# mfkiwl/conan-slam

Hardware: AMD Instinct MI355X
Metric: ekf_update_steps_per_sec (higher is better)
Workload: dtype f32

## Files before the change

conan_slam_amd/_capi.py:

```python
from __future__ import annotations

import ctypes as C
import os
import re

_HERE = os.path.dirname(os.path.abspath(__file__))
LIB_PATH = os.path.join(_HERE, "lib", "libcslam_hip.so")
HEADER_PATH = os.path.join(_HERE, "..", "include", "cslam.h")

OK, ERR_BAD_ARG, ERR_CAPACITY, ERR_HIP, ERR_NO_DEVICE, ERR_ALLOC = 0, 1, 2, 3, 4, 5
FACTOR_OK, FACTOR_FALLBACK, FACTOR_ZEROED, FACTOR_SKIPPED, FACTOR_BAD_IDF, FACTOR_INTERNAL = 0, 1, 2, 4, 8, 16
FACTOR_HEADING_SKIPPED = 32
F32, F64 = 0, 1
Q_LOWER_CHOL_GAIN, Q_PREDICT_NM4, Q_REF_EXACT, Q_TEXTBOOK = 1, 2, 3, 0
STAGE_GATHER, STAGE_FACTOR, STAGE_GAIN, STAGE_DOWNDATE, N_STAGES = 0, 1, 2, 3, 4
STAGE_NAMES = ["gather", "factor", "gain", "downdate"]


class CslamError(RuntimeError):
    def __init__(self, code: int, msg: str):
        super().__init__(f"cslam status {code}: {msg}")
        self.code = code


BATCH_MC_SYMBOLS = ("cslam_ekf_batch_predict_each", "cslam_ekf_batch_get_poses")

LANDMARK_SYMBOLS = ("cslam_ekf_get_landmarks", "cslam_ekf_batch_get_landmarks")
_PROTOTYPES = {
    "cslam_ekf_get_landmarks": [C.c_void_p, C.c_int, C.c_int, C.c_void_p, C.c_void_p, C.c_void_p],
    "cslam_ekf_batch_get_landmarks": [C.c_void_p, C.c_int, C.c_int, C.c_void_p, C.c_void_p, C.c_void_p],
    "cslam_ekf_rows_launches": [C.c_void_p, C.POINTER(C.c_longlong)],
    "cslam_sim_batch_create": [C.c_void_p, C.c_int, C.c_int, C.POINTER(C.c_longlong), C.c_int, C.POINTER(C.c_void_p)],
    "cslam_sim_batch_destroy": [C.c_void_p],
    "cslam_sim_batch_scan": [C.c_void_p, C.c_void_p, C.c_double, C.c_void_p, C.c_longlong, C.POINTER(C.c_int),
                             C.POINTER(C.c_int), C.POINTER(C.c_int)],
    "cslam_sim_batch_get_scan": [C.c_void_p, C.c_int, C.c_void_p, C.c_void_p, C.c_void_p, C.c_void_p],
    "cslam_sim_batch_get_table": [C.c_void_p, C.c_void_p],
    "cslam_sim_batch_set_table": [C.c_void_p, C.c_void_p],
    "cslam_ekf_batch_update_scan": [C.c_void_p, C.c_void_p, C.c_void_p],
    "cslam_ekf_batch_augment_scan": [C.c_void_p, C.c_void_p, C.c_void_p],
    "cslam_pf_best_particle": [C.c_void_p, C.c_int, C.POINTER(C.c_int)] + [C.c_void_p] * 5,
    "cslam_pf_estimate": [C.c_void_p, C.POINTER(C.c_double), C.POINTER(C.c_double)] + [C.c_void_p] * 4,
    "cslam_pf_get_all_features": [C.c_void_p, C.c_void_p],
    "cslam_pf_best_particle_sharded": [C.c_void_p, C.c_void_p, C.c_int, C.POINTER(C.c_longlong)] + [C.c_void_p] * 5,
    "cslam_pf_estimate_sharded": [C.c_void_p, C.c_void_p, C.POINTER(C.c_double), C.POINTER(C.c_double)]
                                 + [C.c_void_p] * 4,
}
PF_ESTIMATE_SYMBOLS = tuple(k for k in _PROTOTYPES if k.startswith("cslam_pf_"))
PF_PICK_MAX, PF_PICK_MIN = 0, 1
SIM_BATCH_SYMBOLS = tuple(k for k in _PROTOTYPES if "sim_batch" in k or k.endswith("_scan"))

SCORE_FIELD_NAMES = ("POSE_N", "POSE_BAD", "POSE_IN", "POSE_ERR2", "POSE_EPHI2", "POSE_NEES",
                     "LM_N", "LM_BAD", "LM_IN", "LM_ERR2", "LM_NEES")
(SCORE_POSE_N, SCORE_POSE_BAD, SCORE_POSE_IN, SCORE_POSE_ERR2, SCORE_POSE_EPHI2, SCORE_POSE_NEES,
 SCORE_LM_N, SCORE_LM_BAD, SCORE_LM_IN, SCORE_LM_ERR2, SCORE_LM_NEES) = range(len(SCORE_FIELD_NAMES))
SCORE_FIELDS = len(SCORE_FIELD_NAMES)
_PROTOTYPES.update({
    "cslam_ekf_batch_score_reset": [C.c_void_p, C.c_int, C.c_double, C.c_double],
    "cslam_ekf_batch_score_set_truth": [C.c_void_p, C.c_void_p, C.c_int],
    "cslam_ekf_batch_score": [C.c_void_p, C.c_void_p],
    "cslam_ekf_batch_score_scan": [C.c_void_p, C.c_void_p, C.c_void_p],
    "cslam_ekf_batch_get_scores": [C.c_void_p, C.c_void_p, C.c_void_p, C.c_int, C.POINTER(C.c_int),
                                   C.POINTER(C.c_longlong)],
})
SCORE_SYMBOLS = tuple(k for k in _PROTOTYPES if "_score" in k)


_PROTOTYPES.update({
    "cslam_pf_associate": [C.c_void_p, C.c_void_p, C.c_int, C.c_void_p, C.c_double, C.c_double],
    "cslam_pf_get_association": [C.c_void_p, C.c_void_p, C.c_void_p, C.c_void_p],
    "cslam_pf_sample_proposal_assoc": [C.c_void_p, C.c_void_p, C.c_int, C.c_void_p, C.c_void_p, C.c_void_p, C.c_double],
    "cslam_pf_feature_update_assoc": [C.c_void_p, C.c_void_p, C.c_int, C.c_void_p, C.c_void_p],
    "cslam_pf_get_stream": [C.c_void_p, C.POINTER(C.c_void_p)],
})
PF_ASSOC_SYMBOLS = tuple(k for k in _PROTOTYPES if k.startswith("cslam_pf_") and "assoc" in k)
PF_ASSOC_FEAT_CHUNK, PF_ASSOC_OBS_CHUNK = 32, 8


def declared_symbols(header_path: str = HEADER_PATH):
    text = open(header_path).read()
    text = re.sub(r"/\*.*?\*/", "", text, flags=re.S)
    return sorted(set(re.findall(r"\b(cslam_[a-z0-9_]+)\s*\(", text)))


# ... 49 lines not shown
```

conan_slam_amd/csrc/cslam_ekf.hip:

```cpp
#include <hip/hip_runtime.h>

#include <algorithm>
#include <atomic>
#include <cfloat>
#include <cmath>
#include <cstdint>
#include <cstdlib>
#include <new>
#include <string>
#include <thread>
#include <vector>

#include "cslam_common.hpp"
#include "device_owners.hpp"
#include "ekf_kernels.hpp"
#include "ekf_kernels_fast.hpp"
#include "ekf_landmark_kernels.hpp"
#include "ekf_lookahead.hpp"
#include "ekf_options.hpp"
#include "ekf_pending_store.hpp"
#include "ekf_pgemm_limbs.hpp"
#include "ekf_pose_kernels.hpp"
#include "ekf_staging.hpp"
#include "host_linalg.hpp"
// ... 16 lines not shown
    for (int i = threadIdx.x; i < 3 * j.m; i += 128)
    {
        if (i < 2 * j.m)
        {
            j.Z_out[i] = j.Z[i];
        }
        else
        {
            j.idf_out[i - 2 * j.m] = j.idf[i - 2 * j.m];
        }
    }
    return true;
}
__global__ void __launch_bounds__(128) ekf_la_wide_f32(LaWideArgs a)
{
    if (la_wide_snapshot(a.snap))
    {
        return;
    }
    ekf_la_wide_body<1, 0>(a);
}
__global__ void __launch_bounds__(128) ekf_la_wide_f32_k64(LaWideArgs a)
{
    if (la_wide_snapshot(a.snap))
    {
        return;
    }
    ekf_la_wide_body<1, 64>(a);
}

__global__ void __launch_bounds__(128) ekf_la_wide_f32_k64m(LaWideArgs a, float* WT)
{
    if (la_wide_snapshot(a.snap))
    {
        return;
    }
    ekf_la_wide_body<1, 64, 1>(a, WT);
}

__global__ void __launch_bounds__(256) ekf_la_blocks_mirror_kernel(LaPrepArgs<float> a, LaMirrorArgs mi)
{
    ekf_la_blocks_mirror_body(a, mi);
}
}

using namespace cslam;

namespace
{

std::atomic<int>& g_engines = ::cslam::live_engines();

constexpr size_t kLdsBudget    = 150 * 1024;

struct EkfBase
{
    explicit EkfBase(const EkfOptions& o) : opt(o) {}
    virtual ~EkfBase() {}
    const EkfOptions opt;
    int         dtype    = CSLAM_F32;
    int         device   = 0;
    int         quirks   = CSLAM_Q_REF_EXACT;
    int         nmax     = 0;
    int         ncap     = 0;
    int         ldp      = 0;
    int         n        = 3;
    int         sync_mode = 1;
    int         pgemm_wgs     = 0;
    Stream      stream_own, stream_b_own, stream_f_own;
    hipStream_t stream   = nullptr;
    hipStream_t stream_b = nullptr;
    long long   la_windows = 0;
    long long   stage_launches = 0;
    long long   rows_launches = 0;

    virtual int init()                                                                        = 0;
    virtual int set_state(const void* X, int n, const void* P, int ldp)                        = 0;
    virtual int get_state(void* X, void* P, int ldp)                                           = 0;
    virtual int get_x(void* X, int cap)                                                        = 0;
    virtual int get_landmarks(int first, int count, void* x, void* pll, void* pvl)             = 0;
    virtual int trace(double* tr)                                                              = 0;
    virtual int predict(double v, double swa, const void* Q, double wb, double dt)             = 0;
    virtual int update(const void* Z, int m, const void* R, const int* idf, int batch, bool on_device) = 0;
    virtual int augment(const void* Z, int q, const void* R)                                   = 0;
    virtual int observe_heading(double phi, int use)                                           = 0;
    virtual int associate(const void* Z, int m, const void* R, double g1, double g2, int* idf_out, int* kind) = 0;
    virtual int factor_status(int* flags, int clear)                                           = 0;
    virtual int set_profiling(int on)                                                          = 0;
    virtual int get_stage_times(double* ms, int* launches)                                     = 0;
    virtual int debug_last_update(void* PHT, void* S, void* G, void* W1, void* V, int* k)      = 0;
    virtual int set_deferred(int max_cols)                                                     = 0;
    virtual int do_flush()                                                                     = 0;
    virtual int resolve_predict()                                                              = 0;
    virtual int sync_all()                                                                     = 0;
    virtual int la_drain()                                                                     = 0;
};

template <typename T>
struct Ekf : EkfBase
{
    using EkfBase::EkfBase;
    DevBuf<T>   dX, dP;
    DevBuf<T>   dPv;
    DevBuf<int> dPoseDone;
    DevBuf<int> dSign;
    DevBuf<T>   dLm;
    PendingCols pend;
    Event      ev_a2b, ev_pgemm;
    T*         last_slot = nullptr;
    struct Workspace
    {
        DevBuf<T> dPHT, dS, dG, dGt, dV, dt_, dScrS, dScrG;
        DevBuf<T> dSub;
        DevBuf<T> dM;
        DevBuf<T> dU;
        DevBuf<T> dWv;
        DevBuf<T> dY;

        int alloc(int ldp, int newk, int wcap, hipStream_t st)
        {
            const size_t kk = (size_t)newk * (newk + 1);
            int          rc = dPHT.alloc_zeroed((size_t)ldp * newk, st);
            if (rc || (rc = dS.alloc(kk)) || (rc = dG.alloc(kk)) || (rc = dSub.alloc((size_t)(3 + 64) * 64)) ||
                (rc = dM.alloc((size_t)3 * 128)) || (rc = dGt.alloc(kk)) || (rc = dScrS.alloc(kk)) ||
                (rc = dScrG.alloc(kk)) || (rc = dV.alloc((size_t)newk)) || (rc = dt_.alloc((size_t)newk)) ||
                (rc = dU.alloc((size_t)newk)) || (rc = dWv.alloc_zeroed((size_t)3 * newk, st)) || (wcap > 0 &&
                (rc = dY.alloc((size_t)newk * wcap))))
// ... 1882 lines not shown
                }
            }
        }
        if (V)
        {
            CSLAM_HIP_TRY(hipMemcpyAsync(V, dbgV ? dbgV : ws.dV.get(), (size_t)k * sizeof(T), hipMemcpyDeviceToHost,
                                         stream));
        }
        CSLAM_HIP_TRY(hipStreamSynchronize(stream));
        return CSLAM_OK;
    }
};

template <typename T>
int Ekf<T>::ensure_tile_list(int tiles)
{
    if (tiles == tiles_built)
    {
        return CSLAM_OK;
    }
    std::vector<int2> h;
    h.reserve((size_t)tiles * (tiles + 1) / 2);
    for (int tj = 0; tj < tiles; tj++)
    {
        for (int ti = tj; ti < tiles; ti++)
        {
            h.push_back(make_int2(ti, tj));
        }
    }
    if (int rc = sync_all())
    {
        return rc;
    }
    DevBuf<int2> list;
    CSLAM_TRY(list.alloc(h.size()));
    dTiles = std::move(list);
    CSLAM_HIP_TRY(hipMemcpy(dTiles.get(), h.data(), h.size() * sizeof(int2), hipMemcpyHostToDevice));
    tiles_built = tiles;
    n_sym_tiles = (int)h.size();
    return CSLAM_OK;
}

template <>
int Ekf<float>::launch_downdate(const float* W, int k, hipStream_t stream)
{
    const int tiles = round_up(n, kTile) / kTile;
    const int k8    = round_up(k, 8);
    int rc = ensure_tile_list(tiles);
    if (rc)
    {
        return rc;
    }
    const dim3 block(256);
    int G = std::min(n_sym_tiles, std::max(1, 2 * (num_cus - la_cus) - (opt.pipeline ? opt.pgemm_spare : 0)));
    if (pgemm_wgs > 0)
    {
        G = std::min(G, pgemm_wgs);
    }
    const bool nt = opt.psym_nt >= 0 ? opt.psym_nt != 0 : (size_t)n_sym_tiles * 65536 > ((size_t)230 << 20);
    if (limbs_take(k8))
    {
        const int    nch  = k8 <= 64 ? 4 : (k8 <= 96 ? 6 : (k8 <= 128 ? 8 : (k8 <= 192 ? 12 : 16)));
        const int    kgs  = 2 * nch;
        const int    rows = round_up(n, kTile);
        const size_t need = (size_t)2 * 3 * kgs * rows * 16;
        if (need > wb_bytes)
        {
            CSLAM_HIP_TRY(hipStreamSynchronize(stream));
            const size_t  cap = (size_t)2 * 3 * 32 * round_up(ncap, kTile) * 16;
            DevBuf<uint4> wb;
            CSLAM_TRY(wb.alloc(cap / sizeof(uint4)));
            dWb      = std::move(wb);
            wb_bytes = cap;
        }
        if ((rc = ensure_tiles_morton(tiles, stream)))
        {
            return rc;
        }
        hipLaunchKernelGGL(ekf_limb_split_kernel, dim3((rows + 255) / 256, kgs), dim3(256), 0, stream, W, ldp, k, rows, kgs,
                           dWb.get());
        limb_parity ^= 1;
#define CSLAM_LAUNCH_PSYM5(MODE, NCH, NP, RR)                                                                          \
    do                                                                                                                 \
    {                                                                                                                  \
        static bool attr_set = false;                                                                                  \
        if (!attr_set)                                                                                                 \
        {                                                                                                              \
            CSLAM_HIP_TRY(hipFuncSetAttribute(reinterpret_cast<const void*>(&ekf_downdate_psym5_bf16<MODE, NCH, NP, RR>), \
                                              hipFuncAttributeMaxDynamicSharedMemorySize, 150 * 1024));               \
            attr_set = true;                                                                                           \
        }                                                                                                              \
        hipLaunchKernelGGL((ekf_downdate_psym5_bf16<MODE, NCH, NP, RR>), dim3(G), block, (size_t)RR * 24576, stream, dP.get(), ldp, \
                           (const uint4*)dWb.get(), rows, (const int2*)dTilesM.get(), (const int*)dSegOff.get(), dTicketX.get() + 8 * limb_parity,  \
                           dTicketX.get() + 8 * (limb_parity ^ 1));                                                          \
    } while (0)
#define CSLAM_LAUNCH_PSYM5R(NCH, RR)                                                                                   \
    do                                                                                                                 \
    {                                                                                                                  \
        if (opt.pgemm_limbs == 6)                                                                                          \
        {                                                                                                              \
            if (nt) { CSLAM_LAUNCH_PSYM5(1, NCH, 6, RR); } else { CSLAM_LAUNCH_PSYM5(0, NCH, 6, RR); }                 \
        }                                                                                                              \
        else                                                                                                           \
        {                                                                                                              \
            if (nt) { CSLAM_LAUNCH_PSYM5(1, NCH, 9, RR); } else { CSLAM_LAUNCH_PSYM5(0, NCH, 9, RR); }                 \
        }                                                                                                              \
    } while (0)
        switch (nch)
        {
        case 4: CSLAM_LAUNCH_PSYM5R(4, 3); break;
        case 6: CSLAM_LAUNCH_PSYM5R(6, 3); break;
        case 8: CSLAM_LAUNCH_PSYM5R(8, 3); break;
        case 12: CSLAM_LAUNCH_PSYM5R(12, 3); break;
        default: CSLAM_LAUNCH_PSYM5R(16, 3); break;
        }
#undef CSLAM_LAUNCH_PSYM5R
#undef CSLAM_LAUNCH_PSYM5
    }
    else if (k8 <= 128 && opt.lower && ldp < 32768)
    {
        launch_parity++;
        const bool xq = opt.xcd_queues != 0 && G >= 64;
        if (xq)
        {
            if ((rc = ensure_tiles_morton(tiles, stream)))
            {
                return rc;
            }
            limb_parity ^= 1;
        }
#define CSLAM_LAUNCH_PSYM4(MODE, NCH, KC)                                                                             \
    hipLaunchKernelGGL((ekf_downdate_psym4_f32<MODE, NCH, KC>), dim3(G), block, 0, stream, dP.get(), ldp, W, ldp, k,         \
                       xq ? (const int2*)dTilesM.get() : (const int2*)dTiles.get(), n_sym_tiles,                                  \
                       xq ? dTicketX.get() + 8 * limb_parity : dTicket.get() + (launch_parity & 1),                              \
                       xq ? dTicketX.get() + 8 * (limb_parity ^ 1) : dTicket.get() + ((launch_parity + 1) & 1),                  \
                       (unsigned long long*)nullptr, xq ? (const int*)dSegOff.get() : (const int*)nullptr, 0u, 0u, 0u, 0u,           \
                       la_sig_add ? la.done.get() : (unsigned*)nullptr, la_sig_add, 1, 0)
        if (k8 <= 64)
        {
            if (nt) { CSLAM_LAUNCH_PSYM4(1, 2, 32); } else { CSLAM_LAUNCH_PSYM4(0, 2, 32); }
        }
        else if (k8 <= 96)
        {
            if (nt) { CSLAM_LAUNCH_PSYM4(1, 4, 24); } else { CSLAM_LAUNCH_PSYM4(0, 4, 24); }
        }
        else
        {
            if (nt) { CSLAM_LAUNCH_PSYM4(1, 4, 32); } else { CSLAM_LAUNCH_PSYM4(0, 4, 32); }
        }
#undef CSLAM_LAUNCH_PSYM4
        la_sig_add = 0;
    }
    else if (opt.lower)
    {
        hipLaunchKernelGGL((ekf_downdate_psym_f32<64, true, false>), dim3(G), block, 0, stream, dP.get(), ldp, W, ldp,
                           k8, dTiles.get(), n_sym_tiles, (long long*)nullptr);
    }
    else
    {
        hipLaunchKernelGGL((ekf_downdate_psym_f32<64, true, true>), dim3(G), block, 0, stream, dP.get(), ldp, W, ldp,
                           k8, dTiles.get(), n_sym_tiles, (long long*)nullptr);
    }
    CSLAM_HIP_TRY(hipGetLastError());
    return CSLAM_OK;
}

template <>
bool Ekf<float>::launch_gain_fast(int k, int n_pad, float* slot, const float* Gt, const float* U, const float* M)
{
    if (k > 128)
    {
        return false;
    }
    hipLaunchKernelGGL((ekf_panel_mfma_f32<false, true>), dim3(n_pad / 32, (k + 31) / 32), dim3(64), 0, stream,
                       ws.dPHT.get(), ldp, n, k, k, Gt, k, U, slot, ldp, dX.get(),
                       fuse_now ? (const float*)dPred.get() : (const float*)nullptr, pp.w, dPv.get(), ldp, M,
                       ws.dWv.get());
    pose_fused_in_gain = (M != nullptr);
    return true;
}

template <>
bool Ekf<float>::launch_corr_fast(int k, const float* Wp, int kc)
{
    const int n_pad = round_up(n, kTile);
    hipLaunchKernelGGL((ekf_panel_mfma_f32<true, false>), dim3(n_pad / 32, (k + 31) / 32), dim3(64), 0, stream, Wp, ldp, n,
                       kc, k, ws.dY.get(), k, nullptr, ws.dPHT.get(), ldp, nullptr);
    return true;
}

template <>
bool Ekf<double>::launch_corr_fast(int k, const double* Wp, int kc)
{
    const int n_pad = round_up(n, kTile);
    hipLaunchKernelGGL((ekf_panel_mfma_f64<true, false>), dim3(n_pad / 16, (k + 15) / 16), dim3(64), 0, stream, Wp, ldp, n, kc,
                       k, ws.dY.get(), k, nullptr, ws.dPHT.get(), ldp, nullptr);
    return true;
}

template <>
bool Ekf<double>::launch_gain_fast(int k, int n_pad, double* slot, const double* Gt, const double* U, const double* M)
// ... 265 lines not shown
    return B(h)->augment(Z, q, R);
}

int cslam_ekf_associate(cslam_ekf_t h, const void* Z, int m, const void* R, double gate1, double gate2, int* idf_out,
                        int* kind_out)
{
    CSLAM_NEED(h);
    if (int rc = B(h)->resolve_predict())
    {
        return rc;
    }
    return B(h)->associate(Z, m, R, gate1, gate2, idf_out, kind_out);
}

int cslam_ekf_observe_heading(cslam_ekf_t h, double phi, int use_heading)
{
    CSLAM_NEED(h);
    return B(h)->observe_heading(phi, use_heading);
}

int cslam_ekf_set_pgemm_workgroups(cslam_ekf_t h, int workgroups)
{
    CSLAM_NEED(h);
    if (workgroups < 0)
    {
        return fail(CSLAM_ERR_BAD_ARG, "set_pgemm_workgroups: negative");
    }
    B(h)->pgemm_wgs = workgroups;
    return CSLAM_OK;
}

int cslam_ekf_lookahead_windows(cslam_ekf_t h, long long* windows)
{
    CSLAM_NEED(h);
    if (!windows)
    {
        return fail(CSLAM_ERR_BAD_ARG, "lookahead_windows: null");
    }
    *windows = B(h)->la_windows;
    return CSLAM_OK;
}

int cslam_ekf_rows_launches(cslam_ekf_t h, long long* launches)
{
    CSLAM_NEED(h);
    if (!launches)
    {
        return fail(CSLAM_ERR_BAD_ARG, "rows_launches: null");
    }
    *launches = B(h)->rows_launches;
    return CSLAM_OK;
}

int cslam_ekf_stage_launches(cslam_ekf_t h, long long* launches)
{
    CSLAM_NEED(h);
    if (!launches)
    {
        return fail(CSLAM_ERR_BAD_ARG, "stage_launches: null");
    }
    *launches = B(h)->stage_launches;
    return CSLAM_OK;
}

int cslam_ekf_get_streams(cslam_ekf_t h, void** chain_stream, void** pgemm_stream)
{
    CSLAM_NEED(h);
    if (chain_stream)
    {
        *chain_stream = reinterpret_cast<void*>(B(h)->stream);
    }
    if (pgemm_stream)
    {
        *pgemm_stream = reinterpret_cast<void*>(B(h)->stream_b);
    }
    return CSLAM_OK;
}

int cslam_ekf_run_many(cslam_ekf_t* handles, int count, int steps, const double* v, const double* swa, const void* Q,
                       double wb, double dt, const void* const* dZ, const int* const* d_idf, int m, const void* R,
                       int batch)
{
    if (!handles || count < 0 || steps < 0 || m < 0 || !R || !Q || (steps > 0 && (!v || !swa)) || (m > 0 && (!dZ || !d_idf)))
    {
        return fail(CSLAM_ERR_BAD_ARG, "run_many: bad arguments");
    }
    for (int i = 0; i < count; i++)
    {
        if (!handles[i] || (m > 0 && (!dZ[i] || !d_idf[i])))
        {
            return fail(CSLAM_ERR_BAD_ARG, "run_many: null handle or input for instance %d", i);
        }
    }
    std::vector<int>         rcs((size_t)count, CSLAM_OK);
    std::vector<std::string> msgs((size_t)count);
    auto                     body = [&](int i) {
        EkfBase*     e     = B(handles[i]);
        const size_t esz   = (e->dtype == CSLAM_F32) ? sizeof(float) : sizeof(double);
        const char*  zbase = m > 0 ? static_cast<const char*>(dZ[i]) : nullptr;
        for (int t = 0; t < steps; t++)
        {
            int rc = e->predict(v[t], swa[t], Q, wb, dt);
            if (!rc && m > 0)
            {
                rc = e->update(zbase + (size_t)t * 2 * m * esz, m, R, d_idf[i] + (size_t)t * m, batch, true);
            }
// ... 79 lines not shown
```

conan_slam_amd/csrc/ekf_kernels_fast.hpp:

```cpp
#pragma once

#include <hip/hip_runtime.h>

#include <type_traits>

#include "ekf_kernels.hpp"

namespace cslam
{

typedef float f32x4 __attribute__((ext_vector_type(4)));
typedef float f32x16 __attribute__((ext_vector_type(16)));

__device__ inline float bcast(float v, int src)
{
    return __int_as_float(__builtin_amdgcn_readlane(__float_as_int(v), src));
}
__device__ inline double bcast(double v, int src)
{
    int lo = __builtin_amdgcn_readlane(__double2loint(v), src);
    int hi = __builtin_amdgcn_readlane(__double2hiint(v), src);
    return __hiloint2double(hi, lo);
}

// ... 2113 lines not shown
    __shared__ __attribute__((aligned(16))) float s_b0[KC * 128];
    __shared__ __attribute__((aligned(16))) float s_a0[KC * 128];
    __shared__ __attribute__((aligned(16))) float s_b1[KC * 128];
    __shared__ __attribute__((aligned(16))) float s_a1[KC * 128];
    __shared__ int2 s_next;

    const int tid  = threadIdx.x;
    const int wave = __builtin_amdgcn_readfirstlane(tid >> 6);
    const int lane = tid & 63;
    const int lj   = lane & 31;
    const int lh   = lane >> 5;
    const int G    = xq ? (int)((gridDim.x - (blockIdx.x & 7u) + 7u) >> 3) : (int)gridDim.x;

    typedef __attribute__((address_space(3))) void* lptr_t;
    typedef unsigned u32x4 __attribute__((ext_vector_type(4)));
    constexpr int kAuxLd = (NTMODE == 1 || NTMODE == 2) ? 2 : ((NTMODE >= 4) ? 16 : 0);
    constexpr int kAuxSt = (NTMODE == 1 || NTMODE == 3 || NTMODE == 6) ? 2 : ((NTMODE == 5) ? 16 : 0);
    const __amdgpu_buffer_rsrc_t rsP =
        __builtin_amdgcn_make_buffer_rsrc(P, 0, BATCH ? p_span : (unsigned)((size_t)ldp * ldp * 4), 0x00020000);
    const __amdgpu_buffer_rsrc_t rsW = __builtin_amdgcn_make_buffer_rsrc(
        const_cast<float*>(W1), 0, BATCH ? w_span : (unsigned)((size_t)k8 * ldw * 4), 0x00020000);
    const unsigned lane_off = (unsigned)(((wave * 32 + 4 * lh) * ldp + 4 * lj) * 4);
    auto tile_base = [&](int2 t) -> unsigned {
        if constexpr (BATCH)
        {
            return (unsigned)(t.x >> 16) * sP + (unsigned)(((size_t)(t.y * 128) * ldp + (t.x & 0xFFFF) * 128) * 4);
        }
        return (unsigned)(((size_t)(t.y * 128) * ldp + t.x * 128) * 4);
    };
    auto row_off   = [&](int r) -> unsigned { return (unsigned)(((r & 3) + 8 * (r >> 2)) * ldp * 4); };
    auto load1     = [&](unsigned tbase, int r) -> f32x4 {
        return __builtin_bit_cast(f32x4, __builtin_amdgcn_raw_buffer_load_b128(rsP, lane_off, tbase + row_off(r), kAuxLd));
    };
    auto store1 = [&](unsigned tbase, int r, f32x4 v) {
        __builtin_amdgcn_raw_buffer_store_b128(__builtin_bit_cast(u32x4, v), rsP, lane_off, tbase + row_off(r), kAuxSt);
    };
    const unsigned dma_lane_off = (unsigned)((lh * ldw + 4 * lj) * 4);
    auto dma_chunk = [&](int2 t, auto C) {
        constexpr int  c    = decltype(C)::value;
        const unsigned ibase = BATCH ? (unsigned)(t.x >> 16) * sW : 0u;
        const unsigned row0  = ibase + (unsigned)((BATCH ? (t.x & 0xFFFF) : t.x) * 128 * 4);
        const unsigned col0  = ibase + (unsigned)(t.y * 128 * 4);
#pragma unroll
        for (int it = 0; it < KC / 8; it++)
        {
            const int      kkb  = it * 8 + wave * 2;
            const unsigned roff = (unsigned)((c * KC + kkb) * ldw * 4);
            lptr_t         db   = (lptr_t)(((c & 1) == 0 ? s_b0 : s_b1) + kkb * 128);
            lptr_t         da   = (lptr_t)(((c & 1) == 0 ? s_a0 : s_a1) + kkb * 128);
            __builtin_amdgcn_raw_ptr_buffer_load_lds(rsW, db, 16, dma_lane_off, roff + row0, 0, 0);
            __builtin_amdgcn_raw_ptr_buffer_load_lds(rsW, da, 16, dma_lane_off, roff + col0, 0, 0);
        }
    };

    f32x16 acc0, acc1, acc2, acc3;
    auto mfma_group = [&](auto B, int g) {
        constexpr int bsel = decltype(B)::value;
        const float*  sB   = bsel == 0 ? s_b0 : s_b1;
        const float*  sA   = bsel == 0 ? s_a0 : s_a1;
        const float4  b    = *reinterpret_cast<const float4*>(&sB[(2 * g + lh) * 128 + 4 * lj]);
        const float   a    = sA[(2 * g + lh) * 128 + wave * 32 + lj];
        acc0               = __builtin_amdgcn_mfma_f32_32x32x2f32(a, b.x, acc0, 0, 0, 0);
        acc1               = __builtin_amdgcn_mfma_f32_32x32x2f32(a, b.y, acc1, 0, 0, 0);
        acc2               = __builtin_amdgcn_mfma_f32_32x32x2f32(a, b.z, acc2, 0, 0, 0);
        acc3               = __builtin_amdgcn_mfma_f32_32x32x2f32(a, b.w, acc3, 0, 0, 0);
    };
    using C0 = std::integral_constant<int, 0>;
    constexpr int kLoadChunkA = (NCH == 2) ? 0 : 1;
    constexpr int kLoadChunkB = (NCH == 2) ? 1 : 2;
    constexpr int kLoadA_g0   = (NCH == 2) ? 8 : 0;

    f32x4 pv[16];

    auto process = [&](auto FIRST, int2 cur, unsigned cbase, unsigned prev_base, int t_next_in, int& t_next_out,
                       int2& nxt_out) -> bool {
        constexpr bool first = decltype(FIRST)::value;
        int2           look   = make_int2(-1, -1);
        int            tk_new = 0;
        int2           nxt    = make_int2(-1, -1);
        bool           have_next = false;
        auto chunk = [&](auto CC) {
            constexpr int c = decltype(CC)::value;
            constexpr int nb_prev = (c == 0) ? ((NCH - 1 == kLoadChunkA ? 8 : 0) + (NCH - 1 == kLoadChunkB ? 8 : 0))
                                             : ((c - 1 == 0 && !first ? 16 : 0) + (c - 1 == kLoadChunkA ? 8 : 0) +
                                                (c - 1 == kLoadChunkB ? 8 : 0));
            if constexpr (c == 0)
            {
                __builtin_amdgcn_s_waitcnt((first || nb_prev == 0) ? 0x0070 : 0xC07F);
            }
            else
            {
                __builtin_amdgcn_s_waitcnt(nb_prev == 0 ? 0x0F70 : (nb_prev == 8 ? 0x0F78 : (nb_prev == 16 ? 0x4F70 : 0x4F78)));
                if (c == 1 && !first && tid == 0)
                {
                    s_next = look;
                }
                __builtin_amdgcn_s_waitcnt(0xC07F);
            }
            __builtin_amdgcn_s_barrier();
            __builtin_amdgcn_sched_barrier(0);
            if constexpr (c == 0)
            {
                if (tid == 0)
                {
                    if (!first)
                    {
                        int tk_raw = t_next_in;
                        asm volatile("" : "+v"(tk_raw));
                        const int tt = 2 * G + tk_raw;
                        if (tt >= 0 && tt < ntiles)
                        {
                            look = tile_list[tt];
                        }
                    }
                    const int zero = 0, one = 1;
                    asm volatile("s_nop 4\n\tglobal_atomic_add %0, %1, %2, %3 sc0" : "=v"(tk_new) : "v"(zero), "v"(one), "s"(ticket) : "memory");
                }
                acc0 = acc1 = acc2 = acc3 = f32x16{0};
            }
            if constexpr (c == 1)
            {
                if (first)
                {
                    nxt = t_next_in < ntiles ? tile_list[t_next_in] : make_int2(-1, -1);
                }
                else
                {
                    const int2 sn = s_next;
                    nxt           = make_int2(__builtin_amdgcn_readfirstlane(sn.x), __builtin_amdgcn_readfirstlane(sn.y));
                }
                have_next = nxt.x >= 0;
                asm volatile("" : "+v"(tk_new));
            }
            if constexpr (c + 1 < NCH)
            {
                dma_chunk(cur, std::integral_constant<int, c + 1>{});
            }
            else
            {
                dma_chunk(have_next ? nxt : cur, C0{});
            }
            __builtin_amdgcn_sched_barrier(0);
            float4 b_cur = make_float4(0.f, 0.f, 0.f, 0.f);
            float  a_cur = 0.f;
            if constexpr (PF)
            {
                const float* sB = (c & 1) == 0 ? s_b0 : s_b1;
                const float* sA = (c & 1) == 0 ? s_a0 : s_a1;
                b_cur           = *reinterpret_cast<const float4*>(&sB[lh * 128 + 4 * lj]);
                a_cur           = sA[lh * 128 + wave * 32 + lj];
            }
#pragma unroll
            for (int g = 0; g < KC / 2; g++)
            {
                if constexpr (PF)
                {
                    const float* sB = (c & 1) == 0 ? s_b0 : s_b1;
                    const float* sA = (c & 1) == 0 ? s_a0 : s_a1;
                    float4       b_nxt = b_cur;
                    float        a_nxt = a_cur;
                    if (g + 1 < KC / 2)
                    {
                        b_nxt = *reinterpret_cast<const float4*>(&sB[(2 * (g + 1) + lh) * 128 + 4 * lj]);
                        a_nxt = sA[(2 * (g + 1) + lh) * 128 + wave * 32 + lj];
                    }
                    acc0  = __builtin_amdgcn_mfma_f32_32x32x2f32(a_cur, b_cur.x, acc0, 0, 0, 0);
                    acc1  = __builtin_amdgcn_mfma_f32_32x32x2f32(a_cur, b_cur.y, acc1, 0, 0, 0);
                    acc2  = __builtin_amdgcn_mfma_f32_32x32x2f32(a_cur, b_cur.z, acc2, 0, 0, 0);
                    acc3  = __builtin_amdgcn_mfma_f32_32x32x2f32(a_cur, b_cur.w, acc3, 0, 0, 0);
                    b_cur = b_nxt;
                    a_cur = a_nxt;
                }
                else
                {
                    mfma_group(std::integral_constant<int, (c & 1)>{}, g);
                }
                if (c == 0 && g < 8 && !first)
                {
                    store1(prev_base, 2 * g, pv[2 * g]);
                    store1(prev_base, 2 * g + 1, pv[2 * g + 1]);
                }
                if (c == kLoadChunkA && g >= kLoadA_g0 && g < kLoadA_g0 + 8)
                {
                    pv[g - kLoadA_g0] = load1(cbase, g - kLoadA_g0);
                }
                if (c == kLoadChunkB && g < 8)
                {
                    pv[g + 8] = load1(cbase, g + 8);
                }
                __builtin_amdgcn_sched_barrier(0);
            }
        };
        chunk(std::integral_constant<int, 0>{});
        chunk(std::integral_constant<int, 1>{});
        if constexpr (NCH == 4)
        {
            chunk(std::integral_constant<int, 2>{});
            chunk(std::integral_constant<int, 3>{});
        }
        asm volatile("" ::: "memory");
#pragma unroll
        for (int r = 0; r < 16; r++)
        {
            pv[r][0] -= acc0[r];
            pv[r][1] -= acc1[r];
            pv[r][2] -= acc2[r];
            pv[r][3] -= acc3[r];
        }
        t_next_out = tk_new;
        nxt_out    = nxt;
        return have_next;
    };

    const int t = xq ? (int)(blockIdx.x >> 3) : (int)blockIdx.x;
    if (blockIdx.x == 0 && tid < (xq ? 8 : 1))
    {
        ticket_reset[tid] = 0;
    }
    if (t >= ntiles)
    {
        return;
    }
    int2     cur   = tile_list[t];
    unsigned cbase = tile_base(cur);
    dma_chunk(cur, C0{});
    if (hwids != nullptr && tid == 0)
    {
        hwids[4 * blockIdx.x]     = __builtin_amdgcn_s_getreg((31 << 11) | 4);
        hwids[4 * blockIdx.x + 1] = __builtin_amdgcn_s_getreg((31 << 11) | 20);
        hwids[4 * blockIdx.x + 2] = __builtin_amdgcn_s_memrealtime();
    }
    int  tk = 0;
    int2 nxt;
    bool hn = process(std::true_type{}, cur, cbase, 0u, t + G, tk, nxt);
    while (hn)
    {
        const unsigned rbase = cbase;
        cur                  = nxt;
        cbase                = tile_base(cur);
        hn                   = process(std::false_type{}, cur, cbase, rbase, tk, tk, nxt);
    }
// ... 42 lines not shown
```

conan_slam_amd/csrc/ekf_options.hpp:

```cpp
#pragma once

#include <algorithm>
#include <cstdlib>
#include <cstring>

namespace cslam
{
inline int env_int(const char* name, int dflt) { const char* s = getenv(name); return s ? atoi(s) : dflt; }
inline int env_flag(const char* name, int dflt) { const char* s = getenv(name); return s ? (atoi(s) ? 1 : 0) : dflt; }

struct EkfOptions
{
    int fuse_predict = 1;
    int fuse_f64     = 1;
    int seq_defer    = 1;
    int lower = 1;
    int pipeline    = 0;
    int pgemm_spare = 16;
    int gather_corr_wide = 1;
    int lookahead    = -1;
    int la_hold_wide = 1;
    int la_k64       = 1;
    int la_wg_signal = 0;
    int la_mirror    = 1;
    int la_fused     = 1;
    int la_stamps    = 0;
    int pgemm_limbs = 0;
    int limbs_kmin  = 65;
    int xcd_queues = 0;
    int psym_nt    = -1;
    int f64_kcm = 16;
    int f64_cb  = 0;

    static EkfOptions from_env()
    {
        EkfOptions o;
        o.fuse_predict     = env_int("CSLAM_FUSE_PREDICT", o.fuse_predict);
        o.fuse_f64         = env_flag("CSLAM_FUSE_F64", o.fuse_f64);
        o.seq_defer        = env_int("CSLAM_SEQ_DEFER", o.seq_defer);
        const char* sv     = getenv("CSLAM_STORAGE");
        o.lower            = (sv && !strcmp(sv, "full")) ? 0 : 1;
        o.pipeline         = env_flag("CSLAM_PIPELINE", o.pipeline);
        o.pgemm_spare      = std::max(0, env_int("CSLAM_PGEMM_SPARE", o.pgemm_spare));
        o.gather_corr_wide = env_flag("CSLAM_GATHER_WIDE", o.gather_corr_wide);
        const int la       = env_int("CSLAM_LOOKAHEAD", o.lookahead);
        o.lookahead        = la > 0 ? 1 : (la < 0 ? -1 : 0);
        o.la_hold_wide     = env_flag("CSLAM_LA_HOLD_WIDE", o.la_hold_wide);
        o.la_k64           = env_flag("CSLAM_LA_K64", o.la_k64);
        o.la_wg_signal     = env_flag("CSLAM_LA_WG_SIGNAL", o.la_wg_signal);
        o.la_mirror        = env_flag("CSLAM_LA_MIRROR", o.la_mirror);
        o.la_fused         = env_flag("CSLAM_LA_FUSED", o.la_fused);
        o.la_stamps        = getenv("CSLAM_LA_STAMPS") ? 1 : 0;
        const int limbs    = env_int("CSLAM_PGEMM_LIMBS", o.pgemm_limbs);
        o.pgemm_limbs      = (limbs == 6 || limbs == 9) ? limbs : 0;
        const int kmin     = env_int("CSLAM_LIMBS_KMIN", o.limbs_kmin);
        o.limbs_kmin       = kmin < 0 ? o.limbs_kmin : std::max(57, kmin);
        o.xcd_queues       = env_flag("CSLAM_XCD_QUEUES", o.xcd_queues);
        o.psym_nt          = env_flag("CSLAM_PSYM_NT", o.psym_nt);
        o.f64_kcm          = std::max(4, std::min(64, (env_int("CSLAM_F64_KCM", o.f64_kcm) + 3) / 4 * 4));
        if (getenv("CSLAM_F64_CB"))
        {
            o.f64_cb = env_int("CSLAM_F64_CB", 0) == 2 ? 2 : 4;
        }
        return o;
    }
};

struct EkfBatchOptions
{
    int wg_signal  = 0;
    int wide_pairs = 2;
    int la_k64     = 1;
    int stamps     = 0;

    static EkfBatchOptions from_env()
    {
        EkfBatchOptions o;
        o.wg_signal  = env_flag("CSLAM_BATCH_WG_SIGNAL", o.wg_signal);
        o.wide_pairs = env_int("CSLAM_BATCH_WIDE_PAIRS", o.wide_pairs) == 1 ? 1 : 2;
        o.la_k64     = env_flag("CSLAM_LA_K64", o.la_k64);
        o.stamps     = getenv("CSLAM_BATCH_STAMPS") ? 1 : 0;
        return o;
    }
};

}
```

conan_slam_amd/ekf.py:

```python
from __future__ import annotations

import ctypes as C

import numpy as np

from . import _capi
from ._capi import (F32, F64, Q_REF_EXACT, Q_TEXTBOOK, check)


def _vp(a: np.ndarray):
    return a.ctypes.data_as(C.c_void_p)


class EKF:
    def __init__(self, max_landmarks: int, dtype=np.float32, device: int = -1, quirks: int = Q_REF_EXACT,
                 sync_mode: bool = True):
        self.dtype = np.dtype(dtype)
        if self.dtype not in (np.dtype(np.float32), np.dtype(np.float64)):
            raise ValueError("dtype must be float32 or float64")
        self._L = _capi.lib()
        self._h = C.c_void_p(None)
        code = F32 if self.dtype == np.float32 else F64
        check(self._L.cslam_ekf_create(C.c_int(max_landmarks), C.c_int(code), C.c_int(device), C.c_int(quirks),
                                       C.byref(self._h)))
# ... 46 lines not shown

    def set_state(self, X, P):
        X = np.ascontiguousarray(X, dtype=self.dtype)
        P = np.asfortranarray(P, dtype=self.dtype)
        n = X.shape[0]
        assert P.shape == (n, n)
        check(self._L.cslam_ekf_set_state(self._h, _vp(X), C.c_int(n), _vp(P), C.c_int(n)))

    def get_state(self):
        n = self.n
        X = np.zeros(n, dtype=self.dtype)
        P = np.zeros((n, n), dtype=self.dtype, order="F")
        check(self._L.cslam_ekf_get_state(self._h, _vp(X), _vp(P), C.c_int(n)))
        return X, P

    def get_x(self):
        n = self.n
        X = np.zeros(n, dtype=self.dtype)
        check(self._L.cslam_ekf_get_x(self._h, _vp(X), C.c_int(n)))
        return X

    def get_p(self):
        return self.get_state()[1]

    X = property(get_x)
    P = property(get_p)

    def trace(self) -> float:
        t = C.c_double(0.0)
        check(self._L.cslam_ekf_trace(self._h, C.byref(t)))
        return t.value

    def synchronize(self):
        check(self._L.cslam_ekf_synchronize(self._h))

    def lookahead_windows(self) -> int:
        w = C.c_longlong(0)
        check(self._L.cslam_ekf_lookahead_windows(self._h, C.byref(w)))
        return w.value

    def streams(self):
        a, b = C.c_void_p(None), C.c_void_p(None)
        check(self._L.cslam_ekf_get_streams(self._h, C.byref(a), C.byref(b)))
        return a.value or 0, b.value or 0

    def stage_launches(self) -> int:
        w = C.c_longlong(0)
        check(self._L.cslam_ekf_stage_launches(self._h, C.byref(w)))
        return w.value

    def rows_launches(self) -> int:
        w = C.c_longlong(0)
        check(self._L.cslam_ekf_rows_launches(self._h, C.byref(w)))
        return w.value

    def landmarks(self, first: int = 1, count: int = None):
        if count is None:
            count = max((self.n - 3) // 2 - first + 1, 0)
        x = np.empty((count, 2), dtype=self.dtype)
        pll = np.empty((count, 4), dtype=self.dtype)
        pvl = np.empty((count, 6), dtype=self.dtype)
        check(self._L.cslam_ekf_get_landmarks(self._h, int(first), int(count), _vp(x), _vp(pll), _vp(pvl)))
        return x, pll.reshape(count, 2, 2).transpose(0, 2, 1).copy(), pvl.reshape(count, 2, 3).transpose(0, 2, 1).copy()

    def factor_status(self, clear: bool = False) -> int:
        f = C.c_int(0)
        check(self._L.cslam_ekf_factor_status(self._h, C.byref(f), C.c_int(1 if clear else 0)))
        return f.value

    def predict(self, v, swa, Q, wb, dt):
        Q = self._mat22(Q)
        check(self._L.cslam_ekf_predict(self._h, C.c_double(float(v)), C.c_double(float(swa)), _vp(Q),
                                        C.c_double(float(wb)), C.c_double(float(dt))))

    def update(self, Z, R, idf, batch: bool = False):
        Z = np.asarray(Z, dtype=self.dtype)
        m = 0 if Z.size == 0 else Z.reshape(2, -1, order="F").shape[1]
        Zc = self._arr(Z) if m else np.zeros(2, dtype=self.dtype)
        R = self._mat22(R)
        idf = np.ascontiguousarray(idf, dtype=np.int32)
        assert idf.shape[0] == m
        idp = idf.ctypes.data_as(C.c_void_p) if m else None
        check(self._L.cslam_ekf_update(self._h, _vp(Zc), C.c_int(m), _vp(R), idp, C.c_int(1 if batch else 0)))

    def update_device(self, dZ_ptr: int, m: int, R, d_idf_ptr: int, batch: bool = True):
        R = self._mat22(R)
        check(self._L.cslam_ekf_update_device(self._h, C.c_void_p(dZ_ptr), C.c_int(m), _vp(R), C.c_void_p(d_idf_ptr),
                                              C.c_int(1 if batch else 0)))

    def augment(self, Z, R):
        Z = np.asarray(Z, dtype=self.dtype)
        q = 0 if Z.size == 0 else Z.reshape(2, -1, order="F").shape[1]
        Zc = self._arr(Z) if q else np.zeros(2, dtype=self.dtype)
        R = self._mat22(R)
        check(self._L.cslam_ekf_augment(self._h, _vp(Zc), C.c_int(q), _vp(R)))

    def observe_heading(self, phi, use_heading: bool = False):
        check(self._L.cslam_ekf_observe_heading(self._h, C.c_double(float(phi)), C.c_int(1 if use_heading else 0)))

    def associate(self, Z, R, gate1, gate2):
        Z = np.asarray(Z, dtype=self.dtype, order="F").reshape(2, -1, order="F")
        R = np.asarray(R, dtype=self.dtype, order="F")
        m = Z.shape[1]
        idf = np.zeros(max(m, 1), dtype=np.int32)
        kind = np.zeros(max(m, 1), dtype=np.int32)
        check(self._L.cslam_ekf_associate(self._h, Z.ctypes.data_as(C.c_void_p), C.c_int(m), R.ctypes.data_as(C.c_void_p),
# ... 228 lines not shown
```

include/cslam.h:

```cpp
#ifndef CSLAM_H
#define CSLAM_H

#ifdef __cplusplus
extern "C" {
#endif

#define CSLAM_VERSION 100

#define CSLAM_OK 0
#define CSLAM_ERR_BAD_ARG 1
#define CSLAM_ERR_CAPACITY 2
#define CSLAM_ERR_HIP 3
#define CSLAM_ERR_NO_DEVICE 4
#define CSLAM_ERR_ALLOC 5
#define CSLAM_FACTOR_OK 0
#define CSLAM_FACTOR_FALLBACK 1
#define CSLAM_FACTOR_ZEROED 2
#define CSLAM_FACTOR_SKIPPED 4
#define CSLAM_FACTOR_INTERNAL 16
#define CSLAM_FACTOR_BAD_IDF 8
#define CSLAM_FACTOR_HEADING_SKIPPED 32

#define CSLAM_F32 0
#define CSLAM_F64 1
// ... 3 lines not shown
#define CSLAM_Q_REF_EXACT 3
#define CSLAM_Q_TEXTBOOK 0

#define CSLAM_STAGE_GATHER 0
#define CSLAM_STAGE_FACTOR 1
#define CSLAM_STAGE_GAIN 2
#define CSLAM_STAGE_DOWNDATE 3
#define CSLAM_N_STAGES 4

typedef struct cslam_ekf* cslam_ekf_t;

const char* cslam_last_error(void);
int cslam_version(void);
int cslam_device_count(int* count);


int cslam_ekf_create(int max_landmarks, int dtype, int device, int quirks, cslam_ekf_t* out);
int cslam_ekf_destroy(cslam_ekf_t h);

int cslam_ekf_set_sync_mode(cslam_ekf_t h, int sync_mode);

int cslam_ekf_set_state(cslam_ekf_t h, const void* X, int n, const void* P, int ldp);
int cslam_ekf_get_state(cslam_ekf_t h, void* X, void* P, int ldp);
int cslam_ekf_get_x(cslam_ekf_t h, void* X, int capacity);
int cslam_ekf_get_n(cslam_ekf_t h, int* n);
int cslam_ekf_get_landmarks(cslam_ekf_t h, int first, int count, void* x, void* pll, void* pvl);
int cslam_ekf_trace(cslam_ekf_t h, double* trace);
int cslam_ekf_synchronize(cslam_ekf_t h);
int cslam_ekf_factor_status(cslam_ekf_t h, int* flags, int clear);

int cslam_ekf_predict(cslam_ekf_t h, double v, double swa, const void* Q, double wb, double dt);

int cslam_ekf_update(cslam_ekf_t h, const void* Z, int m, const void* R, const int* idf, int batch);

int cslam_ekf_update_device(cslam_ekf_t h, const void* dZ, int m, const void* R, const int* d_idf, int batch);

int cslam_ekf_augment(cslam_ekf_t h, const void* Z, int q, const void* R);

int cslam_ekf_observe_heading(cslam_ekf_t h, double phi, int use_heading);

int cslam_ekf_associate(cslam_ekf_t h, const void* Z, int m, const void* R, double gate1, double gate2, int* idf_out,
                        int* kind_out);

int cslam_ekf_set_deferred(cslam_ekf_t h, int max_pending_columns);
int cslam_ekf_flush(cslam_ekf_t h);

int cslam_ekf_get_streams(cslam_ekf_t h, void** chain_stream, void** pgemm_stream);

int cslam_ekf_lookahead_windows(cslam_ekf_t h, long long* windows);

int cslam_ekf_stage_launches(cslam_ekf_t h, long long* launches);

int cslam_ekf_rows_launches(cslam_ekf_t h, long long* launches);

int cslam_ekf_set_pgemm_workgroups(cslam_ekf_t h, int workgroups);

int cslam_ekf_run_many(cslam_ekf_t* handles, int count, int steps, const double* v, const double* swa, const void* Q,
                       double wb, double dt, const void* const* dZ, const int* const* d_idf, int m, const void* R,
                       int batch);

typedef struct cslam_ekf_batch* cslam_ekf_batch_t;
int cslam_ekf_batch_create(int instances, int n_landmarks, int device, int quirks, cslam_ekf_batch_t* out);
int cslam_ekf_batch_destroy(cslam_ekf_batch_t h);
int cslam_ekf_batch_set_state(cslam_ekf_batch_t h, int instance, const float* X, int n, const float* P, int ldp);
int cslam_ekf_batch_get_state(cslam_ekf_batch_t h, int instance, float* X, float* P, int ldp);
int cslam_ekf_batch_run(cslam_ekf_batch_t h, int steps, const double* v, const double* swa, const float* Q, double wb,
                        double dt, const float* const* dZ, const int* const* d_idf, int m, const float* R);
int cslam_ekf_batch_flush(cslam_ekf_batch_t h);
int cslam_ekf_batch_synchronize(cslam_ekf_batch_t h);
int cslam_ekf_batch_trace(cslam_ekf_batch_t h, double* traces );
int cslam_ekf_batch_factor_status(cslam_ekf_batch_t h, int* flags );
int cslam_ekf_batch_info(cslam_ekf_batch_t h, int* instances, int* n, long long* windows);
int cslam_ekf_batch_set_profiling(cslam_ekf_batch_t h, int every);
int cslam_ekf_batch_get_pgemm_time(cslam_ekf_batch_t h, double* ms_sum, int* launches);

int cslam_ekf_batch_create_capacity(int instances, int max_landmarks, int n_landmarks, int device, int quirks,
                                    cslam_ekf_batch_t* out);
int cslam_ekf_batch_predict(cslam_ekf_batch_t h, double v, double swa, const float* Q, double wb, double dt);
int cslam_ekf_batch_predict_each(cslam_ekf_batch_t h, const double* v, const double* swa, const float* Q, double wb,
                                 double dt);
int cslam_ekf_batch_get_poses(cslam_ekf_batch_t h, float* x, float* pvv);
int cslam_ekf_batch_get_landmarks(cslam_ekf_batch_t h, int first, int count, float* x, float* pll, float* pvl);

enum { CSLAM_SCORE_POSE_N, CSLAM_SCORE_POSE_BAD, CSLAM_SCORE_POSE_IN, CSLAM_SCORE_POSE_ERR2 ,
       CSLAM_SCORE_POSE_EPHI2 , CSLAM_SCORE_POSE_NEES ,
       CSLAM_SCORE_LM_N, CSLAM_SCORE_LM_BAD, CSLAM_SCORE_LM_IN, CSLAM_SCORE_LM_ERR2, CSLAM_SCORE_LM_NEES,
       CSLAM_SCORE_FIELDS };
int cslam_ekf_batch_score_reset(cslam_ekf_batch_t h, int series_capacity, double gate_pose, double gate_lm);
int cslam_ekf_batch_score_set_truth(cslam_ekf_batch_t h, const float* lm_true , int count);
int cslam_ekf_batch_score(cslam_ekf_batch_t h, const float* xv_true );
int cslam_ekf_batch_get_scores(cslam_ekf_batch_t h, double* totals ,
                               float* series , int capacity_records, int* records, long long* calls);
int cslam_ekf_batch_observe_heading(cslam_ekf_batch_t h, double phi, int use_heading);
int cslam_ekf_batch_update(cslam_ekf_batch_t h, const float* const* dZ, const int* const* d_idf, int m, const float* R);
int cslam_ekf_batch_augment(cslam_ekf_batch_t h, const float* const* dZn, int q, const float* R);

int cslam_ekf_set_profiling(cslam_ekf_t h, int on);
int cslam_ekf_get_stage_times(cslam_ekf_t h, double* ms_sum, int* launches);

int cslam_ekf_debug_last_update(cslam_ekf_t h, void* PHT, void* S, void* G, void* W1, void* V, int* k);

typedef struct cslam_pf* cslam_pf_t;

int cslam_pf_create(int n_particles, int max_features, int dtype, int device, int quirks, cslam_pf_t* out);
int cslam_pf_destroy(cslam_pf_t h);
int cslam_pf_synchronize(cslam_pf_t h);
// ... 91 lines not shown
```

Measured before the change: 13570.

## Add PF variant of psym4 downdate interleaving DMA pieces with MFMA groups

Adds a prefetch-friendly variant of the f32 psym4 downdate kernel for 96<k<=128. Instead of issuing the whole next-chunk DMA at once, it splits the DMA into eight pieces interleaved with the MFMA groups, and shifts the prev-tile stores and loads later to make room. An optional solo mode halves the workgroup count and pads dynamic LDS so only one workgroup fits per CU. The default mode (2) turns on the interleaved DMA without solo, so the schedule changes for matching k ranges at the risk of extra instruction overhead.

```diff
diff --git a/conan_slam_amd/_capi.py b/conan_slam_amd/_capi.py
--- a/conan_slam_amd/_capi.py
+++ b/conan_slam_amd/_capi.py
@@ -30,6 +30,7 @@
     "cslam_ekf_get_landmarks": [C.c_void_p, C.c_int, C.c_int, C.c_void_p, C.c_void_p, C.c_void_p],
     "cslam_ekf_batch_get_landmarks": [C.c_void_p, C.c_int, C.c_int, C.c_void_p, C.c_void_p, C.c_void_p],
     "cslam_ekf_rows_launches": [C.c_void_p, C.POINTER(C.c_longlong)],
+    "cslam_ekf_solo_launches": [C.c_void_p, C.POINTER(C.c_longlong)],
     "cslam_sim_batch_create": [C.c_void_p, C.c_int, C.c_int, C.POINTER(C.c_longlong), C.c_int, C.POINTER(C.c_void_p)],
     "cslam_sim_batch_destroy": [C.c_void_p],
     "cslam_sim_batch_scan": [C.c_void_p, C.c_void_p, C.c_double, C.c_void_p, C.c_longlong, C.POINTER(C.c_int),
diff --git a/conan_slam_amd/csrc/cslam_ekf.hip b/conan_slam_amd/csrc/cslam_ekf.hip
--- a/conan_slam_amd/csrc/cslam_ekf.hip
+++ b/conan_slam_amd/csrc/cslam_ekf.hip
@@ -92,6 +92,7 @@
 std::atomic<int>& g_engines = ::cslam::live_engines();
 
 constexpr size_t kLdsBudget    = 150 * 1024;
+constexpr size_t kPgemmSoloPadLds = 24 * 1024;
 
 struct EkfBase
 {
@@ -113,6 +114,7 @@
     long long   la_windows = 0;
     long long   stage_launches = 0;
     long long   rows_launches = 0;
+    long long   solo_launches = 0;
 
     virtual int init()                                                                        = 0;
     virtual int set_state(const void* X, int n, const void* P, int ldp)                        = 0;
@@ -2101,7 +2103,10 @@
         return rc;
     }
     const dim3 block(256);
-    int G = std::min(n_sym_tiles, std::max(1, 2 * (num_cus - la_cus) - (opt.pipeline ? opt.pgemm_spare : 0)));
+    const bool pf   = opt.pgemm_solo != 0 && k8 > 96 && k8 <= 128 && opt.lower && ldp < 32768 && !limbs_take(k8);
+    const bool solo = pf && opt.pgemm_solo == 1;
+    int G = std::min(n_sym_tiles,
+                     std::max(1, (solo ? 1 : 2) * (num_cus - la_cus) - (opt.pipeline ? opt.pgemm_spare : 0)));
     if (pgemm_wgs > 0)
     {
         G = std::min(G, pgemm_wgs);
@@ -2193,9 +2198,33 @@
         {
             if (nt) { CSLAM_LAUNCH_PSYM4(1, 4, 24); } else { CSLAM_LAUNCH_PSYM4(0, 4, 24); }
         }
+        else if (!pf)
+        {
+            if (nt) { CSLAM_LAUNCH_PSYM4(1, 4, 32); } else { CSLAM_LAUNCH_PSYM4(0, 4, 32); }
+        }
         else
         {
-            if (nt) { CSLAM_LAUNCH_PSYM4(1, 4, 32); } else { CSLAM_LAUNCH_PSYM4(0, 4, 32); }
+            const size_t pad = solo ? kPgemmSoloPadLds : 0;
+#define CSLAM_LAUNCH_PSYM4_SOLO(MODE)                                                                                  \
+    do                                                                                                                 \
+    {                                                                                                                  \
+        static bool attr_set = false;                                                                                  \
+        if (!attr_set)                                                                                                 \
+        {                                                                                                              \
+            CSLAM_HIP_TRY(hipFuncSetAttribute(reinterpret_cast<const void*>(&ekf_downdate_psym4_f32<MODE, 4, 32, true, false>), \
+                                              hipFuncAttributeMaxDynamicSharedMemorySize, (int)kPgemmSoloPadLds));      \
+            attr_set = true;                                                                                           \
+        }                                                                                                              \
+        hipLaunchKernelGGL((ekf_downdate_psym4_f32<MODE, 4, 32, true, false>), dim3(G), block, pad, stream, dP.get(), ldp, W, ldp, k, \
+                           xq ? (const int2*)dTilesM.get() : (const int2*)dTiles.get(), n_sym_tiles,                          \
+                           xq ? dTicketX.get() + 8 * limb_parity : dTicket.get() + (launch_parity & 1),                      \
+                           xq ? dTicketX.get() + 8 * (limb_parity ^ 1) : dTicket.get() + ((launch_parity + 1) & 1),          \
+                           (unsigned long long*)nullptr, xq ? (const int*)dSegOff.get() : (const int*)nullptr, 0u, 0u, 0u, 0u, \
+                           la_sig_add ? la.done.get() : (unsigned*)nullptr, la_sig_add, 1, 0);                              \
+    } while (0)
+            if (nt) { CSLAM_LAUNCH_PSYM4_SOLO(1); } else { CSLAM_LAUNCH_PSYM4_SOLO(0); }
+#undef CSLAM_LAUNCH_PSYM4_SOLO
+            solo_launches++;
         }
 #undef CSLAM_LAUNCH_PSYM4
         la_sig_add = 0;
@@ -2567,6 +2596,17 @@
     return CSLAM_OK;
 }
 
+int cslam_ekf_solo_launches(cslam_ekf_t h, long long* launches)
+{
+    CSLAM_NEED(h);
+    if (!launches)
+    {
+        return fail(CSLAM_ERR_BAD_ARG, "solo_launches: null");
+    }
+    *launches = B(h)->solo_launches;
+    return CSLAM_OK;
+}
+
 int cslam_ekf_stage_launches(cslam_ekf_t h, long long* launches)
 {
     CSLAM_NEED(h);
diff --git a/conan_slam_amd/csrc/ekf_kernels_fast.hpp b/conan_slam_amd/csrc/ekf_kernels_fast.hpp
--- a/conan_slam_amd/csrc/ekf_kernels_fast.hpp
+++ b/conan_slam_amd/csrc/ekf_kernels_fast.hpp
@@ -2189,6 +2189,16 @@
             __builtin_amdgcn_raw_ptr_buffer_load_lds(rsW, da, 16, dma_lane_off, roff + col0, 0, 0);
         }
     };
+    auto dma_piece = [&](int2 t, auto C, int j) {
+        constexpr int  c     = decltype(C)::value;
+        const unsigned ibase = BATCH ? (unsigned)(t.x >> 16) * sW : 0u;
+        const unsigned from  = (j & 1) == 0 ? ibase + (unsigned)((BATCH ? (t.x & 0xFFFF) : t.x) * 128 * 4)
+                                            : ibase + (unsigned)(t.y * 128 * 4);
+        const int      kkb   = (j >> 1) * 8 + wave * 2;
+        const unsigned roff  = (unsigned)((c * KC + kkb) * ldw * 4);
+        float*         buf   = (j & 1) == 0 ? ((c & 1) == 0 ? s_b0 : s_b1) : ((c & 1) == 0 ? s_a0 : s_a1);
+        __builtin_amdgcn_raw_ptr_buffer_load_lds(rsW, (lptr_t)(buf + kkb * 128), 16, dma_lane_off, roff + from, 0, 0);
+    };
 
     f32x16 acc0, acc1, acc2, acc3;
     auto mfma_group = [&](auto B, int g) {
@@ -2206,6 +2216,8 @@
     constexpr int kLoadChunkA = (NCH == 2) ? 0 : 1;
     constexpr int kLoadChunkB = (NCH == 2) ? 1 : 2;
     constexpr int kLoadA_g0   = (NCH == 2) ? 8 : 0;
+    constexpr int kMemG0 = PF ? KC / 4 : 0;
+    static_assert(!PF || (NCH == 4 && KC == 32), "PF: 8 DMA pieces, then 8 k-pairs of stores / loads per chunk");
 
     f32x4 pv[16];
 
@@ -2269,13 +2281,11 @@
                 have_next = nxt.x >= 0;
                 asm volatile("" : "+v"(tk_new));
             }
-            if constexpr (c + 1 < NCH)
-            {
-                dma_chunk(cur, std::integral_constant<int, c + 1>{});
-            }
-            else
-            {
-                dma_chunk(have_next ? nxt : cur, C0{});
+            using CN        = std::integral_constant<int, (c + 1 < NCH) ? c + 1 : 0>;
+            const int2 dsrc = (c + 1 < NCH) ? cur : (have_next ? nxt : cur);
+            if constexpr (!PF)
+            {
+                dma_chunk(dsrc, CN{});
             }
             __builtin_amdgcn_sched_barrier(0);
             float4 b_cur = make_float4(0.f, 0.f, 0.f, 0.f);
@@ -2312,18 +2322,26 @@
                 {
                     mfma_group(std::integral_constant<int, (c & 1)>{}, g);
                 }
-                if (c == 0 && g < 8 && !first)
-                {
-                    store1(prev_base, 2 * g, pv[2 * g]);
-                    store1(prev_base, 2 * g + 1, pv[2 * g + 1]);
-                }
-                if (c == kLoadChunkA && g >= kLoadA_g0 && g < kLoadA_g0 + 8)
-                {
-                    pv[g - kLoadA_g0] = load1(cbase, g - kLoadA_g0);
-                }
-                if (c == kLoadChunkB && g < 8)
-                {
-                    pv[g + 8] = load1(cbase, g + 8);
+                if constexpr (PF)
+                {
+                    if (g < KC / 4)
+                    {
+                        dma_piece(dsrc, CN{}, g);
+                    }
+                }
+                const int gm = g - kMemG0;
+                if (c == 0 && gm >= 0 && gm < 8 && !first)
+                {
+                    store1(prev_base, 2 * gm, pv[2 * gm]);
+                    store1(prev_base, 2 * gm + 1, pv[2 * gm + 1]);
+                }
+                if (c == kLoadChunkA && gm >= kLoadA_g0 && gm < kLoadA_g0 + 8)
+                {
+                    pv[gm - kLoadA_g0] = load1(cbase, gm - kLoadA_g0);
+                }
+                if (c == kLoadChunkB && gm >= 0 && gm < 8)
+                {
+                    pv[gm + 8] = load1(cbase, gm + 8);
                 }
                 __builtin_amdgcn_sched_barrier(0);
             }
diff --git a/conan_slam_amd/csrc/ekf_options.hpp b/conan_slam_amd/csrc/ekf_options.hpp
--- a/conan_slam_amd/csrc/ekf_options.hpp
+++ b/conan_slam_amd/csrc/ekf_options.hpp
@@ -29,6 +29,7 @@
     int limbs_kmin  = 65;
     int xcd_queues = 0;
     int psym_nt    = -1;
+    int pgemm_solo = 2;
     int f64_kcm = 16;
     int f64_cb  = 0;
 
@@ -57,6 +58,7 @@
         o.limbs_kmin       = kmin < 0 ? o.limbs_kmin : std::max(57, kmin);
         o.xcd_queues       = env_flag("CSLAM_XCD_QUEUES", o.xcd_queues);
         o.psym_nt          = env_flag("CSLAM_PSYM_NT", o.psym_nt);
+        o.pgemm_solo       = std::max(0, std::min(2, env_int("CSLAM_PGEMM_SOLO", o.pgemm_solo)));
         o.f64_kcm          = std::max(4, std::min(64, (env_int("CSLAM_F64_KCM", o.f64_kcm) + 3) / 4 * 4));
         if (getenv("CSLAM_F64_CB"))
         {
diff --git a/conan_slam_amd/ekf.py b/conan_slam_amd/ekf.py
--- a/conan_slam_amd/ekf.py
+++ b/conan_slam_amd/ekf.py
@@ -122,6 +122,11 @@
     def rows_launches(self) -> int:
         w = C.c_longlong(0)
         check(self._L.cslam_ekf_rows_launches(self._h, C.byref(w)))
+        return w.value
+
+    def solo_launches(self) -> int:
+        w = C.c_longlong(0)
+        check(self._L.cslam_ekf_solo_launches(self._h, C.byref(w)))
         return w.value
 
     def landmarks(self, first: int = 1, count: int = None):
diff --git a/include/cslam.h b/include/cslam.h
--- a/include/cslam.h
+++ b/include/cslam.h
@@ -79,6 +79,8 @@
 int cslam_ekf_stage_launches(cslam_ekf_t h, long long* launches);
 
 int cslam_ekf_rows_launches(cslam_ekf_t h, long long* launches);
+
+int cslam_ekf_solo_launches(cslam_ekf_t h, long long* launches);
 
 int cslam_ekf_set_pgemm_workgroups(cslam_ekf_t h, int workgroups);
 
```

After: 14040 (median of 4 runs). +3.5%, better.
